# argsim/argsim

Measured on AMD Instinct MI355X. Metric: sentences/sec per ELBO step, higher is better.
Workload: dtype f32; 1 GPU; BASELINE configs[1]: 1xMI355X fp32, latent_dim 128, vocab 8k, seq_len 64, batch 256 per GPU; FULL synthetic Zipf batches, dim_emb 512, 3 layers, step 20000; global_batch=256, seq_len=64, parallelism=dp1, gru=persistent

## Files before the change

### argsim_amd/csrc/ctx.h

```cpp
#pragma once
#include "../../include/argsim_vae.h"
#include "kernels.h"

#include <fcntl.h>
#include <sys/file.h>
#include <unistd.h>

#include <algorithm>
#include <cmath>
#include <cstdio>
#include <cstring>
#include <string>
#include <vector>

#pragma GCC visibility push(hidden)
namespace avae { namespace host {

struct ParamEntry {
    std::string name;
    int64_t offset;
    int ndim;
    int64_t shape[4];
    int g16;
    int bucket;
// ... 7 lines not shown
struct avae_ctx {
    avae_config cfg{};
    int device = 0;
    hipStream_t stream = nullptr;
    std::string err;
    std::vector<avae::host::ParamEntry> params;
    int64_t numel = 0;
    std::vector<std::pair<int64_t, int64_t>> buckets;
    float *P = nullptr, *G = nullptr, *M = nullptr, *Vv = nullptr;
    int64_t step = 0;
    avae_grad_hook hook = nullptr; void* hook_user = nullptr;
    std::vector<int> hook_pending;
    int persistent = 1;
    bool first_step_checked = false;
    int gru_ablate = 0, gru_force_slow = 0, gru_stagger = 0, gru_item = 2;
    int skinny = 1;
    int score_plan[4] = {0, 0, 0, 0};
    const int* expect_ptr[3] = {nullptr, nullptr, nullptr}; int expect_val[3] = {0, 0, 0};
    int compact = 2;
    int skip_pad = 1;
    int shared_device = 0; int lock_fd = -1;
    int dyn_split = 1;
    int dyn_thin = 1;
    int enc_top1 = 1;
    int table_l1 = 1;
    int bf16_act = 1;
    int bf16_sv = 1;
    int bf16_tn = 1;
    int logits16 = 1;
    int bf16_nt8 = 1;
    int bf16_direct = 0;
    int gru_spec = 2;
    int gru_ring = 1;
    int bwd_rs = 2;
    int knn_chunk = 0;
    int agg_chunk = 0;
    int ward_form = 0;
    int probe_chunk = 0;
    int gru_bf16 = 1;
    int64_t oE = 0, oKout = 0, oBout = 0, oWmu = 0, oBmu = 0, oWlv = 0, oBlv = 0, oWex = 0, oBex = 0;
    std::vector<avae::host::GruP> enc;
    std::vector<avae::host::GruP> dec;
    float* losses = nullptr;
    float* acc = nullptr;
    int* errw = nullptr;
    unsigned* counters = nullptr;
    float* scratch = nullptr;
    int64_t scratch_n = 0;
    char* ws = nullptr; size_t ws_cap = 0;
    int B = 0, Ss = 0, St = 0;
    int timing = 0, timing_on = 0;
    unsigned short *bfA = nullptr, *bfB = nullptr; size_t bfA_cap = 0, bfB_cap = 0;
    float* slab = nullptr; size_t slab_floats = 0;
    unsigned short* bfP = nullptr; size_t bfP_cap = 0;
    struct Stamp { hipEvent_t a, b; int cls; double flops; const int* dyn; int dyn_max; };
    std::vector<Stamp> stamps; size_t stamps_used = 0;
    int32_t* hint_dev = nullptr; volatile int32_t* hint_host = nullptr;
    const int32_t *cnt_src = nullptr, *cnt_tgt = nullptr;
};

#pragma GCC visibility push(hidden)
namespace avae { namespace host {

#define AV_CHECK(expr)                                                                              \
    do { hipError_t e_ = (expr); if (e_ != hipSuccess) {                                            \
        char b_[512]; snprintf(b_, sizeof b_, "%s:%d: %s -> %s", __FILE__, __LINE__, #expr, hipGetErrorString(e_)); \
        h->err = b_; return 1; } } while (0)
#define AV_TRY(expr) do { int r_ = (expr); if (r_) return r_; } while (0)

inline int fail(avae_ctx* h, const std::string& m) { h->err = m; return 1; }

#define AV_GRU(expr)                                                                                                \
    do { hipError_t e_ = (expr);                                                                                    \
         if (e_ == hipErrorCooperativeLaunchTooLarge)                                                               \
             return fail(h, "persistent GRU kernel: its workgroups cannot all be resident on this device at once (occupancy query x CU count < grid); " \
                            "run with avae_set_option(\"persistent\", 0)");                                         \
         if (e_ != hipSuccess) { char b_[512]; snprintf(b_, sizeof b_, "%s:%d: %s -> %s", __FILE__, __LINE__, #expr, hipGetErrorString(e_)); \
             h->err = b_; return 1; } } while (0)

struct DeviceTurn {
    avae_ctx* h; bool held = false;
    explicit DeviceTurn(avae_ctx* h_) : h(h_) {
        if (!h->shared_device || !h->persistent) return;
        if (h->lock_fd < 0) {
            char path[64]; snprintf(path, sizeof path, "/tmp/argsim_vae_dev%d.lock", h->device);
            h->lock_fd = open(path, O_CREAT | O_RDWR, 0666);
        }
        if (h->lock_fd >= 0 && flock(h->lock_fd, LOCK_EX) == 0) held = true;
    }
    ~DeviceTurn() { if (held) { (void)hipStreamSynchronize(h->stream); (void)flock(h->lock_fd, LOCK_UN); } }
};
// ... 10 lines not shown
        s = &h->stamps[h->stamps_used++];
        s->cls = cls; s->flops = flops; s->dyn = dyn; s->dyn_max = dyn_max;
        (void)hipEventRecord(s->a, h->stream);
    }
    ~Timed() { if (s) (void)hipEventRecord(s->b, h->stream); }
};

struct Ws {
    int32_t *src_tm, *lens_src, *lens_tgt, *lead, *gold, *rank, *cidx, *ntok, *pred;
    float *emb_src, *emb_tgt, *ew, *dew;
    std::vector<float*> e_gi, e_hs, e_sv[2], e_hp[2];
    std::vector<float*> d_gi, d_hd, d_sv, d_hp;
    float *hpick, *mu, *lv, *z, *eps, *kld, *h0;
    float *xlast, *gib, *svb, *dgib, *dghb, *dxl;
    float *hc, *ho, *logits;
    float *loss_samp, *errt_samp;
    float *dho, *dhc, *dhd[2], *dgi_d, *dgh_d, *dh0, *carry, *dh0sum, *dz, *dmu, *dlv, *dhpick;
    float *dhs[2], *dgi_e, *dgh_e, *demb_src, *demb_tgt;
    std::vector<unsigned short*> e_hs16, d_hd16, e_hp16[2], d_hp16;
    std::vector<char> act_e, act_d, acth_e, acth_d;
    std::vector<unsigned short*> x16_e, x16_d;
    const unsigned short* x16_kept_e(int i) const { return x16_valid ? x16_e[i] : nullptr; }
    const unsigned short* x16_kept_d(int i) const { return x16_valid ? x16_d[i] : nullptr; }
    bool x16_valid = false;
    unsigned short *dgi16_d, *dgh16_d, *dgi16_e, *dgh16_e;
    int32_t* scat;
    int32_t *grp_src, *grp_tgt;
    int32_t *tokrow_src, *tokrow_tgt;
    float* xbuf; size_t xbuf_floats;
    int32_t *ord_perm[3], *ord_slens[3]; int ord_T[3], ord_cpj[3]; bool ord_ok[3];
    int32_t *map_src, *nact_src, *nsrc; bool compact;
    int32_t *map_tgt, *nact_tgt, *ntgt; bool compact_d;
    int Bx;
    int bx_enc() const { return compact ? Bx : 0; }
    int bx_dec() const { return compact_d ? Bx : 0; }
};

struct Bump {
    char* base; size_t off = 0;
    template <class T> T* take(size_t n) {
        off = (off + 255) & ~(size_t)255;
        T* p = base ? reinterpret_cast<T*>(base + off) : nullptr;
        off += n * sizeof(T);
        return p;
    }
    template <class T> T* opt(bool on, size_t n) { return on ? take<T>(n) : nullptr; }
};

struct Pair { const float* A; const float* B; float* C; const float* bias; };

struct GemmCall {
    const float* A; int lda; bool a_mc;
    const float* B; int ldb; bool b_nc;
    float* C; int ldc;
    int M, N, K;
    float alpha = 1.f; const float* bias = nullptr; int accumulate = 0;
    const int* dyn = nullptr; int dyn_kind = 0;
    const Pair* pair = nullptr;
    bool wgrad = false;
    bool allow_atomic = false;
    bool rows_are_batch = false;
    int thin = -1, split_k = 0;
    const unsigned short* A16 = nullptr; const unsigned short* B16 = nullptr;
    unsigned short* keep_a16 = nullptr;
    unsigned short* c16 = nullptr;

// ... 78 lines not shown
```

### argsim_amd/csrc/handle.cpp

```cpp
#include "ctx.h"

using namespace avae;
using namespace avae::host;

static std::string g_create_err;

namespace avae { namespace host {

int grow_scratch(avae_ctx* h, size_t need, const char* what)
{
    if (h->scratch_n >= (int64_t)need) return 0;
    AV_CHECK(hipStreamSynchronize(h->stream));
    if (h->scratch) AV_CHECK(hipFree(h->scratch));
    h->scratch = nullptr; h->scratch_n = 0;
    if (hipMalloc(reinterpret_cast<void**>(&h->scratch), need) != hipSuccess) {
        (void)hipGetLastError();
        h->scratch = nullptr;
        char b_[256]; snprintf(b_, sizeof b_, "%s: %.0f MB of scratch could not be allocated on the device", what, (double)need / 1048576.0);
        return fail(h, b_);
    }
    h->scratch_n = (int64_t)need;
    return 0;
}

// ... 189 lines not shown
    if (!base) return fail(h, "bad tensor kind");
    float* flat = base + e->offset;
    int64_t n = e->shape[0] * e->shape[1] * e->shape[2] * e->shape[3];
    if (!e->g16) {
        AV_CHECK(hipMemcpyAsync(get ? buf : flat, get ? flat : buf, n * sizeof(float), hipMemcpyDeviceToDevice, h->stream));
    } else {
        int D = h->cfg.dim_emb, cols = (int)(e->ndim == 2 ? e->shape[1] : 1);
        if (get) AV_CHECK(g16_permute(h->stream, buf, flat, D, cols, false));
        else     AV_CHECK(g16_permute(h->stream, flat, buf, D, cols, true));
    }
    return 0;
}
int avae_get_tensor(avae_handle h, const char* name, int kind, float* buf) { return xfer_tensor(h, name, kind, buf, true); }
int avae_set_tensor(avae_handle h, const char* name, int kind, const float* buf) { return xfer_tensor(h, name, kind, const_cast<float*>(buf), false); }

int avae_get_step(avae_handle h, int64_t* s) { if (!h || !s) return 1; *s = h->step; return 0; }
int avae_set_step(avae_handle h, int64_t s) { if (!h) return 1; h->step = s; return 0; }

int avae_set_grad_hook(avae_handle h, avae_grad_hook hook, void* user) { if (!h) return 1; h->hook = hook; h->hook_user = user; return 0; }

int avae_set_option(avae_handle h, const char* key, int value)
{
    if (!h || !key) return 1;
    if (!strcmp(key, "persistent")) { h->persistent = value; return 0; }
    if (!strcmp(key, "gru_item")) { h->gru_item = value; return 0; }
    if (!strcmp(key, "gru_stagger")) { h->gru_stagger = value; return 0; }
    if (!strcmp(key, "gru_force_slow")) { h->gru_force_slow = value; return 0; }
    if (!strcmp(key, "gru_bf16")) { h->gru_bf16 = value != 0; return 0; }
    if (!strcmp(key, "bwd_rs")) { h->bwd_rs = value; return 0; }
    if (!strcmp(key, "dyn_split")) { h->dyn_split = value != 0; return 0; }
    if (!strcmp(key, "shared_device")) { h->shared_device = value != 0; return 0; }
    if (!strcmp(key, "gru_spec")) { h->gru_spec = value; return 0; }
    if (!strcmp(key, "gru_ring")) { h->gru_ring = value != 0; return 0; }
    if (!strcmp(key, "bf16_nt8")) { h->bf16_nt8 = value != 0; return 0; }
    if (!strcmp(key, "logits16")) { h->logits16 = value != 0; return 0; }
    if (!strcmp(key, "bf16_direct")) { h->bf16_direct = value != 0; return 0; }
    if (!strcmp(key, "bf16_tn")) { h->bf16_tn = value != 0; return 0; }
    if (!strcmp(key, "bf16_sv")) { h->bf16_sv = value != 0; return 0; }
    if (!strcmp(key, "bf16_act")) { h->bf16_act = value != 0; return 0; }
    if (!strcmp(key, "table_l1")) { h->table_l1 = value != 0; return 0; }
    if (!strcmp(key, "enc_top1")) { h->enc_top1 = value != 0; return 0; }
    if (!strcmp(key, "dyn_thin")) { h->dyn_thin = value != 0; return 0; }
    if (!strcmp(key, "skip_pad")) { h->skip_pad = value != 0; return 0; }
    if (!strcmp(key, "compact")) { h->compact = value; return 0; }
    if (!strcmp(key, "skinny")) { h->skinny = value; return 0; }
    if (!strcmp(key, "knn_chunk")) { if (value < 0) return fail(h, "knn_chunk must be >= 0"); h->knn_chunk = value; return 0; }
    if (!strcmp(key, "agg_chunk")) { if (value < 0) return fail(h, "agg_chunk must be >= 0"); h->agg_chunk = value; return 0; }
    if (!strcmp(key, "ward_form")) { if (value < 0 || value > 2) return fail(h, "ward_form must be 0 (planner), 1 (one-workgroup) or 2 (launch-per-merge)"); h->ward_form = value; return 0; }
    if (!strcmp(key, "probe_chunk")) { if (value < 0) return fail(h, "probe_chunk must be >= 0"); h->probe_chunk = value; return 0; }
    if (!strcmp(key, "gru_ablate")) {
        if (value && !gru_diag_build()) return fail(h, "gru_ablate needs the diagnostic build of libargsim_vae.so (make -C argsim_amd/csrc DIAG=1)");
        h->gru_ablate = value; return 0;
    }
    if (!strcmp(key, "timing")) { h->timing = value; h->timing_on = value; h->stamps_used = 0; return 0; }
    if (!strcmp(key, "timing_pause")) { h->timing = value ? 0 : h->timing_on; return 0; }
    return fail(h, "unknown option");
}
int avae_timing_collect(avae_handle h, double* out)
{
    if (!h || !out) return 1;
    AV_CHECK(hipStreamSynchronize(h->stream));
    for (int i = 0; i < 9; ++i) out[i] = 0.0;
    std::vector<std::pair<const int*, int>> seen;
    for (size_t i = 0; i < h->stamps_used; ++i) {
        float ms = 0.f;
        AV_CHECK(hipEventElapsedTime(&ms, h->stamps[i].a, h->stamps[i].b));
// ... 17 lines not shown
```

### argsim_amd/csrc/hooks.cpp

```cpp
#include "ctx.h"

using namespace avae;
using namespace avae::host;

extern "C" {

int avae_debug_team_batch(int32_t B) { return B > 0 ? gru_team_batch(B) : 0; }
int avae_debug_gemm_plan(const int32_t* in, int32_t n, int32_t* out)
{
    if (!in || !out || n < 0) return 1;
    for (int r = 0; r < n; ++r, in += 19, out += 15) {
        const GemmShape s{in[0] != 0, in[1] != 0, in[2], in[3], in[4], in[5], in[6], in[7], in[8], in[9], in[10], in[11] != 0, in[12] != 0,
                          in[13] != 0, in[14] != 0, in[15], in[16] != 0, in[17] != 0, in[18] != 0};
        const GemmPlan p = gemm_plan(s);
        out[0] = p.n;
        for (int i = 0; i < 2; ++i) {
            const GemmLaunch l = i < p.n ? p.launch[i] : GemmLaunch{0, 0, 0, 0, 0, 0, 0};
            const int32_t f[7] = {l.row0, l.rows, l.thin, l.split_k, l.accumulate, l.zero, l.dyn};
            std::copy(f, f + 7, out + 1 + 7 * i);
        }
    }
    return 0;
}
int avae_debug_gemm_call(avae_handle h, int a_mc, int b_nc, const float* A, const float* Bm, float* Cm, const float* bias, int M, int N, int K,
// ... 41 lines not shown
                     pair ? other : nullptr, pair ? other : nullptr, nullptr, nullptr};
    const GemmF32Form f = gemm_f32_form(a_mc != 0, b_nc != 0, g);
    const int32_t v[8] = {f.tile, f.fast, f.db, f.persist, (int32_t)f.gx, (int32_t)f.gy, (int32_t)f.gz, f.err != hipSuccess};
    std::copy(v, v + 8, out);
    return 0;
}
int avae_debug_score_plan(avae_handle h, int32_t out[4])
{
    if (!h || !out) return 1;
    for (int i = 0; i < 4; ++i) out[i] = h->score_plan[i];
    return 0;
}
int avae_debug_present_ids(avae_handle h, int32_t out[2])
{
    if (!h || !out) return 1;
    AV_CHECK(hipStreamSynchronize(h->stream));
    out[0] = out[1] = -1;
    if (h->cnt_src) AV_CHECK(hipMemcpy(&out[0], h->cnt_src, sizeof(int), hipMemcpyDeviceToHost));
    if (h->cnt_tgt) AV_CHECK(hipMemcpy(&out[1], h->cnt_tgt, sizeof(int), hipMemcpyDeviceToHost));
    return 0;
}
int avae_debug_train_ce(avae_handle h, float* out, int32_t max_n, int32_t* n_out)
{
    if (!h || !out || !n_out) return 1;
    if (h->B < 1) return fail(h, "avae_debug_train_ce: no training forward has run on this handle");
    Ws w;
    AV_TRY(get_ws(h, w, h->B, h->Ss, h->St, true));
    int n = 0;
    AV_CHECK(hipMemcpyAsync(&n, w.ntok, sizeof(int), hipMemcpyDeviceToHost, h->stream));
    AV_CHECK(hipStreamSynchronize(h->stream));
    n = std::min(n, (int)max_n);
    AV_CHECK(hipMemcpyAsync(out, w.loss_samp, (size_t)n * sizeof(float), hipMemcpyDeviceToDevice, h->stream));
    *n_out = n;
    return 0;
}
int avae_debug_timing(avae_handle h, double* out, int max_n, int* n)
{
    if (!h || !out || !n) return 1;
    AV_CHECK(hipStreamSynchronize(h->stream));
    *n = (int)std::min<size_t>(h->stamps_used, (size_t)max_n);
    std::vector<std::pair<const int*, int>> seen;
    for (int i = 0; i < *n; ++i) {
        float ms = 0.f;
        AV_CHECK(hipEventElapsedTime(&ms, h->stamps[i].a, h->stamps[i].b));
        double f = 1.0;
        AV_TRY(dyn_fraction(h, h->stamps[i], seen, &f));
        const double fl = h->stamps[i].flops * f;
        out[3 * i] = h->stamps[i].cls; out[3 * i + 1] = ms; out[3 * i + 2] = fl;
    }
    return 0;
}
int avae_debug_stamps(avae_handle h, unsigned long long* out)
{
    if (!h || !out) return 1;
    AV_CHECK(hipStreamSynchronize(h->stream));
    AV_CHECK(hipMemcpy(out, h->errw + 16, 32 * sizeof(unsigned long long), hipMemcpyDeviceToHost));
    AV_CHECK(hipMemset(h->errw + 16, 0, 32 * sizeof(unsigned long long)));
    return 0;
}
int avae_debug_gemm(avae_handle h, int a_mc, int b_nc, const float* A, const float* Bm, float* Cm, const float* bias,
                    int M, int N, int K, int lda, int ldb, int ldc, float alpha, int accumulate, int split_k)
{
    if (!h) return 1;
    GemmCall c{A, lda, a_mc != 0, Bm, ldb, b_nc != 0, Cm, ldc, M, N, K};
    c.alpha = alpha; c.bias = bias; c.accumulate = accumulate;
    return gemm(h, c.form(split_k == -3 ? 3 : (split_k < 0 ? 1 : (split_k >= 1000 ? 2 : 0)), split_k < 0 ? 1 : (split_k >= 1000 ? split_k - 1000 : split_k)));
// ... 203 lines not shown
```

### argsim_amd/csrc/kernels.h

```cpp
#pragma once
#include <hip/hip_runtime.h>
#include <stdint.h>

#include "gemm_plan.h"

namespace avae {

struct GemmArgs {
    const float* A; const float* B; float* C; const float* bias;
    int M, N, K, lda, ldb, ldc;
    float alpha;
    int accumulate;
    int split_k;
    const int* dyn; int dyn_kind;
    int dyn_expect;
    int thin;
    const float* A2; const float* B2; float* C2; const float* bias2;
    float* slab = nullptr; size_t slab_floats = 0;
    unsigned short* c16 = nullptr;
    int nt8 = 1;
};
hipError_t gemm_f32(hipStream_t st, bool a_mc, bool b_nc, const GemmArgs& g);
struct GemmF32Form { int tile; bool fast, db, persist; unsigned gx, gy, gz; hipError_t err; };
GemmF32Form gemm_f32_form(bool a_mc, bool b_nc, const GemmArgs& g);
// ... 81 lines not shown
hipError_t gru_bwd_rs_launch(hipStream_t st, const GruArgs& a, const GruPlan& p);
hipError_t gru_fwd_team_launch(hipStream_t st, const GruArgs& a, const GruPlan& p);
hipError_t gru_bwd_team_launch(hipStream_t st, const GruArgs& a, const GruPlan& p);
hipError_t gru_reg_launch(hipStream_t st, const GruArgs& a, bool fwd, int grid, bool need_resident);
hipError_t gru_fwd_item_launch(hipStream_t st, const GruArgs& a, int grid);
hipError_t gru_first_step_fwd(hipStream_t st, const float* gi, const float* bR, float* h_out, int ldo, float* sv, int B, int D, const int32_t* lens = nullptr);
hipError_t gru_first_step_bwd(hipStream_t st, const float* dh, int ldd, const float* sv, float* dgi, float* dgh, int B, int D, const int32_t* lens = nullptr);
bool gru_diag_build();

struct PrepArgs {
    const int32_t* src; const int32_t* tgt;
    int B, Ss, St, eos, bos;
    int train; float keepwd; uint64_t seed; const uint8_t* keep_mask;
    int32_t* src_tm;
    int32_t* lens_src;
    int32_t* lens_tgt;
    int32_t* lead;
    int32_t* gold;
    int32_t* rank;
    int32_t* cidx;
    int32_t* ntok;
    float* zero2;
    int32_t* chunk_counts;
};
constexpr int kPrepChunks = 1024;
hipError_t prep_ids(hipStream_t st, const PrepArgs& p);

hipError_t embed_gather(hipStream_t st, const float* E, const int32_t* ids, float* out, int n, int D, int V);
hipError_t embed_scatter_add2(hipStream_t st, float* dE, const int32_t* ids0, const float* dout0, int n0, const int32_t* ids1,
                              const float* dout1, int n1, int D, int V, int32_t* scratch);
bool id_groups_supported(int V);
inline size_t id_groups_ints(size_t n, size_t V) { return 4 * V + 2 + n + (n / 32 + V + 1) + 2 * V + 4; }
hipError_t id_groups_build(hipStream_t st, const int32_t* ids, int n, int V, int32_t* scratch, bool lists);
const int32_t* id_groups_rank(int32_t* scratch, int n, int V);
const int32_t* id_groups_uid(int32_t* scratch, int n, int V);
const int32_t* id_groups_count(int32_t* scratch, int n, int V);
hipError_t rank_rows(hipStream_t st, int32_t* out, const int32_t* ids, const int32_t* rank, int n, int V);
hipError_t rows_gather_ranked(hipStream_t st, float* dst, const float* src, const int32_t* ids, const int32_t* rank, int n, int W, int V);
hipError_t rows_group_sum(hipStream_t st, float* dst, const int32_t* ids, const float* src, int n, int W, int V, int32_t* scratch);
hipError_t rows_add_indexed(hipStream_t st, float* dst, const float* src, const int32_t* uid, const int32_t* nuniq, int n_max, int D);
inline size_t embed_scatter_scratch_ints(size_t n, size_t V) { return 4 * V + 2 + n + (n / 32 + V + 1); }
struct RowOrder { const int32_t* lens; int add, T, cpj; int32_t* perm; int32_t* slens; };
hipError_t row_order(hipStream_t st, const RowOrder* orders, int n, int Breal, int B, int S, int32_t* steps_sum = nullptr, int sum_rows = 0);
hipError_t rows_gather(hipStream_t st, float* dst, const float* src, const int32_t* idx, const int32_t* n_dev, int n_max, int D, const int32_t* map = nullptr);
hipError_t rows_expand(hipStream_t st, float* dst, const float* src, const int32_t* rank, int rows, int D, const int32_t* map = nullptr);
hipError_t pick_last(hipStream_t st, float* h, const float* hs, const int32_t* lens, int B, int W, const int32_t* map = nullptr);
hipError_t pick_last16(hipStream_t st, float* h, const unsigned short* hs16, const int32_t* lens, int B, int W, const int32_t* map = nullptr);
hipError_t pick_last_add(hipStream_t st, float* dhs, const float* d, const int32_t* lens, int B, int W, const int32_t* map = nullptr);
hipError_t row_map(hipStream_t st, const int32_t* lens, int add, int S, int B, int32_t* map, int32_t* nact, int32_t* count);
hipError_t zero_rows_dyn(hipStream_t st, float* X, const int32_t* count, int rows_max, int W);
hipError_t pick_last_bwd(hipStream_t st, float* dhs, const float* dh, const int32_t* lens, int S, int B, int W);

hipError_t latent_fwd(hipStream_t st, const float* mu, const float* lv, const float* eps_in, float* eps_out, float* z,
                      float* kld, int n, int train, uint64_t seed, float free_bits, float* acc);
hipError_t latent_bwd(hipStream_t st, const float* dz, const float* mu, const float* lv, const float* eps_used,
                      float* dmu, float* dlv, int B, int R, float coef, float free_bits);

struct CeArgs {
    float* logits;
    const int32_t* gold;
    const int32_t* cidx;
    const int32_t* n_dev;
    int n_max, V;
    int write_grad; float inv_n;
    float* loss_samp; float* errt_samp; int32_t* pred;
    float* loss_acc;
// ... 163 lines not shown
```

### argsim_amd/csrc/model.cpp

```cpp
#include "ctx.h"

using namespace avae;

namespace avae { namespace host {

static bool phantom_batch(const avae_ctx* h, int B)
{
    return h->compact && h->skip_pad && h->persistent && h->cfg.dim_emb == 512 && gru_team_batch(B) > B;
}
bool use_table(const avae_ctx* h, int rows, int B)
{
    if (!h->table_l1 || !id_groups_supported(h->cfg.dim_tgt)) return false;
    return rows >= h->cfg.dim_tgt || (rows >= 1024 && phantom_batch(h, B));
}

void layout(avae_ctx* h, Bump& b, Ws& w, int B, int Ss, int St, bool train)
{
    const int D = h->cfg.dim_emb, V = h->cfg.dim_tgt, R = h->cfg.dim_rep, L = h->cfg.rnn_layers;
    const size_t T = St + 1, rs = (size_t)Ss * B, rt = T * B;
    w.src_tm = b.take<int32_t>(rs); w.lens_src = b.take<int32_t>(B); w.lens_tgt = b.take<int32_t>(B);
    w.lead = b.take<int32_t>(rt); w.gold = b.take<int32_t>(rt); w.rank = b.take<int32_t>(rt);
    w.cidx = b.take<int32_t>(rt); w.ntok = b.take<int32_t>(4 + kPrepChunks); w.pred = b.take<int32_t>(rt);
    w.emb_src = b.take<float>(rs * D); w.emb_tgt = b.take<float>(rt * D);
    const bool tab_s = use_table(h, (int)rs, B), tab_t = use_table(h, (int)rt, B);
// ... 363 lines not shown
    AV_CHECK(row_map(h->stream, w.lens_tgt, 1, T, B, w.map_tgt, w.nact_tgt, w.ntgt));
    w.compact_d = true;
    return 0;
}
int build_compact_dec(avae_ctx* h, Ws& w, int B, int T)
{
    w.compact = false; w.compact_d = false;
    h->expect_ptr[0] = h->expect_ptr[1] = h->expect_ptr[2] = nullptr;
    if (!h->compact || h->compact == 3 || !h->persistent || T < 2 || !use_table(h, T * B, B)) return 0;
    if (w.Bx == B || !w.ord_ok[2]) return 0;
    GruArgs q{};
    gru_common(h, w, q, 1, T, B, 3 * h->cfg.dim_emb, h->cfg.dim_emb, nullptr, w.Bx);
    if (!gru_plan(q, true, true).full()) return 0;
    AV_CHECK(row_map(h->stream, w.lens_tgt, 1, T, B, w.map_tgt, w.nact_tgt, w.ntgt));
    w.compact_d = true;
    return 0;
}

static int run_encoder(avae_ctx* h, Ws& w, int B, int Ss, bool save)
{
    const int D = h->cfg.dim_emb, V = h->cfg.dim_tgt, L = h->cfg.rnn_layers;
    const int rs = Ss * B;
    const bool table = use_table(h, rs, B);
    h->cnt_src = table ? id_groups_count(w.grp_src, rs, V) : nullptr;
    const int32_t* const cdyn = w.compact ? w.nsrc : nullptr;
    const int32_t* const cmap = w.compact ? w.map_src : nullptr;
    if (!table) AV_CHECK(embed_gather(h->stream, h->P + h->oE, w.src_tm, w.emb_src, rs, D, V));
    const float* x = w.emb_src; int In = D;
    for (int i = 0; i < L; ++i) {
        const GruP& p = h->enc[i];
        const bool top1 = i == L - 1 && top_one_step(h);
        if (i == 0 && table) {
            const int32_t* cnt = id_groups_count(w.grp_src, rs, V);
            AV_CHECK(id_groups_build(h->stream, w.src_tm, rs, V, w.grp_src, save));
            AV_CHECK(rows_gather(h->stream, w.emb_src, h->P + h->oE, id_groups_uid(w.grp_src, rs, V), cnt, std::min(V, rs), D));
            AV_TRY(gemm(h, nt(w.emb_src, D, h->P + p.W, D, w.ew, 6 * D, std::min(V, rs), 6 * D, D).biased(h->P + p.bW).rows(cnt)));
        } else if (i > 0 && w.act_e[i - 1]) {
            AV_TRY(gemm_bf16_pre(h, nt(nullptr, In, h->P + p.W, In, w.e_gi[i], 6 * D, rs, top1 ? 3 * D : 6 * D, In).a16(w.e_hs16[i - 1]).biased(h->P + p.bW).rows(cdyn)));
        } else {
        AV_TRY(gemm(h, nt(x, In, h->P + p.W, In, w.e_gi[i], 6 * D, rs, top1 ? 3 * D : 6 * D, In).biased(h->P + p.bW).rows(cdyn).keep(save ? w.x16_e[i] : nullptr)));
        }
        GruArgs a{};
        gru_common(h, w, a, top1 ? 1 : 2, Ss, B, 6 * D, 2 * D, w.lens_src, w.bx_enc());
        const bool table0 = i == 0 && table, indirect = table0 && gru_plan(a, true, h->persistent != 0).form == GruForm::team;
        if (indirect) AV_CHECK(rank_rows(h->stream, w.tokrow_src, w.src_tm, id_groups_rank(w.grp_src, rs, V), rs, V));
        else if (table0) AV_CHECK(rows_gather_ranked(h->stream, w.e_gi[0], w.ew, w.src_tm, id_groups_rank(w.grp_src, rs, V), rs, 6 * D, V));
        for (int d = 0; d < a.njobs; ++d) {
            GruJob& j = a.job[d];
            j.gi = (indirect ? w.ew : w.e_gi[i]) + d * 3 * D;
            j.gi_rows = indirect ? w.tokrow_src : nullptr;
            j.R = h->P + p.R + (int64_t)d * 3 * D * D;
            j.bR = h->P + p.bR + d * 3 * D;
            j.h0 = nullptr;
            j.hs = w.e_hs[i] + d * D;
            j.sv = save ? w.e_sv[d][i] : nullptr;
            j.hp = save ? w.e_hp[d][i] : nullptr;
            j.reverse = d;
        }
        attach_sv16(h, a, save);
        if (w.e_hs16[i] && tn16_ok(h, 3 * D, D) && both_team_bf16(h, a, save)) {
            w.act_e[i] = 1; w.acth_e[i] = 1;
            for (int d = 0; d < a.njobs; ++d) { a.job[d].hs16 = w.e_hs16[i] + d * D; a.job[d].hp16 = w.e_hp16[d][i]; }
        }
        attach_order(h, w, a, true, top1 ? 1 : 0);
        a.rowmap = cmap;
        a.spec = spec_pick(h);
        { Timed t(h, 1, 2.0 * a.njobs * Ss * (double)B * D * 3 * D);
// ... 10 lines not shown
    }
    if (w.act_e[L - 1]) AV_CHECK(pick_last16(h->stream, w.hpick, w.e_hs16[L - 1], w.lens_src, B, 2 * D, cmap));
    else
    AV_CHECK(pick_last(h->stream, w.hpick, w.e_hs[L - 1], w.lens_src, B, 2 * D, cmap));
    if (top_one_step(h))
        AV_CHECK(gru_first_step_fwd(h->stream, w.gib, h->P + h->enc[L - 1].bR + 3 * D, w.hpick + D, 2 * D, save ? w.svb : nullptr, B, D, w.lens_src));
    return 0;
}

static int run_latent(avae_ctx* h, Ws& w, int B, bool train, uint64_t seed, const float* eps)
{
    const int D = h->cfg.dim_emb, R = h->cfg.dim_rep;
    {
        const Pair lv{w.hpick, h->P + h->oWlv, w.lv, h->P + h->oBlv};
        AV_TRY(gemm(h, nn(w.hpick, 2 * D, h->P + h->oWmu, R, w.mu, R, B, R, 2 * D).biased(h->P + h->oBmu).with(&lv)));
    }
    AV_CHECK(latent_fwd(h->stream, w.mu, w.lv, eps, w.eps, w.z, w.kld, B * R, train ? 1 : 0, seed, h->cfg.free_bits, nullptr));
    return 0;
}

int run_decoder_rnn(avae_ctx* h, Ws& w, int B, int T, const float* state_in, int64_t state_stride, bool save, const int32_t* ids0, bool compact, const int32_t* share_rows, int share_n)
{
    const int32_t* const cdyn = compact ? w.ntgt : nullptr;
    const int32_t* const cmap = compact ? w.map_tgt : nullptr;
    const int D = h->cfg.dim_emb, L = h->cfg.rnn_layers;
    const int rt = T * B;
    const float* x = w.emb_tgt;
    h->cnt_tgt = ids0 ? id_groups_count(w.grp_tgt, rt, h->cfg.dim_tgt) : nullptr;
    for (int i = 0; i < L; ++i) {
        const GruP& p = h->dec[i];
        if (i == 0 && ids0) {
            const int V = h->cfg.dim_tgt;
            const int32_t* cnt = id_groups_count(w.grp_tgt, rt, V);
            AV_CHECK(id_groups_build(h->stream, ids0, rt, V, w.grp_tgt, save));
            AV_CHECK(rows_gather(h->stream, w.emb_tgt, h->P + h->oE, id_groups_uid(w.grp_tgt, rt, V), cnt, std::min(V, rt), D));
            AV_TRY(gemm(h, nt(w.emb_tgt, D, h->P + p.W, D, w.ew, 3 * D, std::min(V, rt), 3 * D, D).biased(h->P + p.bW).rows(cnt)));
        } else if (i == 0 && share_rows) {
            AV_TRY(gemm(h, nt(x, D, h->P + p.W, D, w.d_gi[0], 3 * D, share_n, 3 * D, D).biased(h->P + p.bW)));
        } else if (i > 0 && w.act_d[i - 1]) {
            AV_TRY(gemm_bf16_pre(h, nt(nullptr, D, h->P + p.W, D, w.d_gi[i], 3 * D, rt, 3 * D, D).a16(w.d_hd16[i - 1]).biased(h->P + p.bW).rows(cdyn)));
        } else {
        AV_TRY(gemm(h, nt(x, D, h->P + p.W, D, w.d_gi[i], 3 * D, rt, 3 * D, D).biased(h->P + p.bW).rows(cdyn).keep(save ? w.x16_d[i] : nullptr)));
        }
        GruArgs a{};
        gru_common(h, w, a, 1, T, B, 3 * D, D, nullptr, compact ? w.Bx : 0);
        GruJob& j = a.job[0];
        const bool table0 = i == 0 && ids0, indirect = table0 && gru_plan(a, true, h->persistent != 0).form == GruForm::team;
        if (indirect) AV_CHECK(rank_rows(h->stream, w.tokrow_tgt, ids0, id_groups_rank(w.grp_tgt, rt, h->cfg.dim_tgt), rt, h->cfg.dim_tgt));
        else if (table0) AV_CHECK(rows_gather_ranked(h->stream, w.d_gi[0], w.ew, ids0, id_groups_rank(w.grp_tgt, rt, h->cfg.dim_tgt), rt, 3 * D, h->cfg.dim_tgt));
        j.gi = indirect ? w.ew : w.d_gi[i]; j.gi_rows = indirect ? w.tokrow_tgt : nullptr;
        if (i == 0 && share_rows) j.gi_rows = share_rows;
        j.R = h->P + p.R; j.bR = h->P + p.bR;
        j.h0 = state_in + state_stride * i;
        j.hs = w.d_hd[i];
        j.sv = save ? w.d_sv[i] : nullptr;
        j.hp = save ? w.d_hp[i] : nullptr;
        j.reverse = 0;
        attach_sv16(h, a, save);
        if (w.d_hp16[i] && tn16_ok(h, 3 * D, D) && both_team_bf16(h, a, save)) {
            if (i < L - 1) { w.act_d[i] = 1; j.hs16 = w.d_hd16[i]; }
            w.acth_d[i] = 1; j.hp16 = w.d_hp16[i];
        }
        if (T > 1) attach_order(h, w, a, true, 2);
        a.rowmap = cmap;
        a.spec = spec_pick(h);
        { Timed t(h, 1, 2.0 * T * (double)B * D * 3 * D);
          DeviceTurn turn(h);
          AV_GRU(gru_forward(h->stream, a, h->persistent != 0)); }
        x = w.d_hd[i];
    }
    return 0;
}

static int forward(avae_ctx* h, Ws& w, const int32_t* src, const int32_t* tgt, int B, int Ss, int St, bool train,
            uint64_t seed, const uint8_t* keep_mask, const float* eps, float inv_n)
{
    const int D = h->cfg.dim_emb, V = h->cfg.dim_tgt, R = h->cfg.dim_rep;
    const int T = St + 1, rt = T * B;
    Sched sc = schedule(h);
    PrepArgs p = prep_from_ws(w);
    p.src = src; p.tgt = tgt; p.B = B; p.Ss = Ss; p.St = St; p.eos = h->cfg.eos; p.bos = h->cfg.bos;
    p.train = train ? 1 : 0; p.keepwd = sc.keepwd; p.seed = seed; p.keep_mask = keep_mask;
    AV_CHECK(prep_ids(h->stream, p));
    AV_TRY(build_row_orders(h, w, B, Ss, T, true));
    AV_TRY(build_compact(h, w, B, Ss, T, train));
    AV_TRY(run_encoder(h, w, B, Ss, train));
    AV_TRY(run_latent(h, w, B, train, seed, eps));
    AV_TRY(gemm(h, nn(w.z, R, h->P + h->oWex, D, w.h0, D, B, D, R).biased(h->P + h->oBex).batch_rows()));
    if (use_table(h, rt, B)) AV_TRY(run_decoder_rnn(h, w, B, T, w.h0, 0, train, w.lead, w.compact_d));
    else {
        AV_CHECK(embed_gather(h->stream, h->P + h->oE, w.lead, w.emb_tgt, rt, D, V));
        AV_TRY(run_decoder_rnn(h, w, B, T, w.h0, 0, train));
    }
    AV_TRY(run_logits_ce(h, w, rt, train, inv_n));
    float beta = h->cfg.kl_beta;
    AV_CHECK(finalize_losses(h->stream, h->losses, w.loss_samp, w.ntok, rt, w.kld, B * R, h->cfg.free_bits, 1.f / ((float)B * R), sc.anneal * beta));
    return 0;
}

int run_logits_ce(avae_ctx* h, Ws& w, int rt, bool train, float inv_n)
{
    const int D = h->cfg.dim_emb, V = h->cfg.dim_tgt, L = h->cfg.rnn_layers;
    AV_CHECK(rows_gather(h->stream, w.hc, w.d_hd[L - 1], w.cidx, w.ntok, rt, D, w.compact_d ? w.map_tgt : nullptr));
    AV_TRY(gemm(h, nn(w.hc, D, h->P + h->oKout, D, w.ho, D, rt, D, D).biased(h->P + h->oBout).rows(w.ntok)));
    CeArgs c{};
    c.logits = w.logits; c.gold = w.gold; c.cidx = w.cidx; c.n_dev = w.ntok; c.n_max = rt; c.V = V;
    c.write_grad = train ? 1 : 0; c.inv_n = inv_n;
    if (train && h->cfg.compute_dtype == 1 && (V & 7) == 0) {
        AV_TRY(grow_bf16(h, &h->bfP, &h->bfP_cap, (size_t)rt * V));
        c.grad16 = h->bfP;
        if (h->logits16 && !h->bf16_direct && gemm_bf16_c16_takes(rt, V, D, w.ntok, h->bf16_nt8)) c.logits16 = 1;
    }
    GemmCall lg = nt(w.ho, D, h->P + h->oE, D, w.logits, V, rt, V, D).scaled(1.f / sqrtf((float)D)).rows(w.ntok);
    if (c.logits16) lg.form(0).c16 = h->bfP;
    AV_TRY(gemm(h, lg));
    c.loss_samp = w.loss_samp; c.errt_samp = w.errt_samp; c.pred = w.pred; c.loss_acc = nullptr;
    AV_CHECK(softmax_ce(h->stream, c));
    return 0;
// ... 335 lines not shown
```

### argsim_amd/csrc/ops.hip

```cpp
#include <algorithm>
#include "kernels.h"
#include "mfma_tile.h"
#include "reduce_dev.h"
#include "sample_dev.h"

namespace avae {


__device__ __forceinline__ bool prep_kept(const PrepArgs& p, int i)
{
    const int t = i / p.B, b = i - t * p.B;
    return t == 0 || p.tgt[(size_t)b * p.St + t - 1] != p.eos;
}
__device__ __forceinline__ int block_sum256(int v, int* red)
{
    v = wave_sum(v);
    if ((threadIdx.x & 63) == 0) red[threadIdx.x >> 6] = v;
    __syncthreads();
    const int s = red[0] + red[1] + red[2] + red[3];
    __syncthreads();
    return s;
}
__global__ __launch_bounds__(256) void prep_ids_kernel(PrepArgs p, int per, int nchunks)
{
// ... 262 lines not shown
        return hipGetLastError();
    }
    Scatter2 a{dE, ids0, dout0, n0, ids1, dout1, n1, D, V, scratch, scratch + V, scratch + 2 * V, scratch + 3 * V + 1, scratch + 4 * V + 2, scratch + 4 * V + 2 + n, nullptr, nullptr, nullptr};
    hipError_t e = zero_fill(st, scratch, sizeof(int32_t) * 2 * (size_t)V);
    if (e != hipSuccess) return e;
    const int blocks = (n + kScatterTok - 1) / kScatterTok;
    hipLaunchKernelGGL(scatter_hist_kernel, dim3(blocks), dim3(256), 0, st, a);
    hipLaunchKernelGGL(scatter_scan_kernel, dim3(1), dim3(1024), 0, st, a);
    hipLaunchKernelGGL(scatter_fill_kernel, dim3(blocks), dim3(256), 0, st, a);
    hipLaunchKernelGGL(scatter_reduce_kernel, dim3(std::min((n / 4 + V + 3) / 4, 4096)), dim3(256), 0, st, a);
    return hipGetLastError();
}

static Scatter2 id_groups_view(const int32_t* ids, int n, int V, int32_t* scratch)
{
    int32_t* rank = scratch + 4 * (size_t)V + 2 + n + ((size_t)n / kScatterSeg + V + 1);
    return Scatter2{nullptr, ids, nullptr, n, nullptr, nullptr, 0, 0, V, scratch, scratch + V, scratch + 2 * V, scratch + 3 * V + 1,
                    scratch + 4 * V + 2, scratch + 4 * (size_t)V + 2 + n, rank, rank + V, rank + 2 * (size_t)V};
}
const int32_t* id_groups_rank(int32_t* scratch, int n, int V) { return id_groups_view(nullptr, n, V, scratch).rank; }
const int32_t* id_groups_uid(int32_t* scratch, int n, int V) { return id_groups_view(nullptr, n, V, scratch).uid; }
const int32_t* id_groups_count(int32_t* scratch, int n, int V) { return id_groups_view(nullptr, n, V, scratch).nuniq; }
bool id_groups_supported(int V) { return V <= kScatterLdsV; }
hipError_t id_groups_build(hipStream_t st, const int32_t* ids, int n, int V, int32_t* scratch, bool lists)
{
    if (n <= 0 || V > kScatterLdsV) return hipErrorInvalidValue;
    Scatter2 a = id_groups_view(ids, n, V, scratch);
    hipError_t e = zero_fill(st, scratch, sizeof(int32_t) * 2 * (size_t)V);
    if (e != hipSuccess) return e;
    const int blocks = (n + kScatterTok - 1) / kScatterTok;
    hipLaunchKernelGGL(scatter_hist_kernel, dim3(blocks), dim3(256), 0, st, a);
    hipLaunchKernelGGL(scatter_scan_kernel, dim3(1), dim3(1024), 0, st, a);
    if (lists) hipLaunchKernelGGL(scatter_fill_kernel, dim3(blocks), dim3(256), 0, st, a);
    return hipGetLastError();
}
__global__ __launch_bounds__(256) void rows_gather_ranked_kernel(float* __restrict__ dst, const float* __restrict__ src,
                                                                 const int32_t* __restrict__ ids, const int32_t* __restrict__ rank, int n, int W, int V)
{
    const int lane = threadIdx.x & 63, wpb = blockDim.x >> 6;
    for (int row = blockIdx.x * wpb + (threadIdx.x >> 6); row < n; row += gridDim.x * wpb) {
        int id = ids[row];
        id = id < 0 ? 0 : (id >= V ? V - 1 : id);
        const float4* s = reinterpret_cast<const float4*>(src + (size_t)rank[id] * W);
        float4* d = reinterpret_cast<float4*>(dst + (size_t)row * W);
        for (int c = lane; c < W / 4; c += 64) d[c] = s[c];
    }
}
__global__ __launch_bounds__(256) void rank_rows_kernel(int32_t* __restrict__ out, const int32_t* __restrict__ ids, const int32_t* __restrict__ rank, int n, int V)
{
    for (int t = blockIdx.x * 256 + threadIdx.x; t < n; t += gridDim.x * 256) {
        int id = ids[t];
        id = id < 0 ? 0 : (id >= V ? V - 1 : id);
        out[t] = rank[id];
    }
}
hipError_t rank_rows(hipStream_t st, int32_t* out, const int32_t* ids, const int32_t* rank, int n, int V)
{
    if (n <= 0) return hipSuccess;
    hipLaunchKernelGGL(rank_rows_kernel, dim3(std::min((n + 255) / 256, 2048)), dim3(256), 0, st, out, ids, rank, n, V);
    return hipGetLastError();
}
hipError_t rows_gather_ranked(hipStream_t st, float* dst, const float* src, const int32_t* ids, const int32_t* rank, int n, int W, int V)
{
    if (n <= 0) return hipSuccess;
    if (W & 3) return hipErrorInvalidValue;
    hipLaunchKernelGGL(rows_gather_ranked_kernel, dim3(std::min((n + 3) / 4, 8192)), dim3(256), 0, st, dst, src, ids, rank, n, W, V);
// ... 827 lines not shown
```

### argsim_amd/lib.py

```python
import ctypes as C
import os
import subprocess

_HERE = os.path.dirname(os.path.abspath(__file__))
LIB_PATH = os.path.join(_HERE, 'libargsim_vae.so')
CSRC = os.path.join(_HERE, 'csrc')


def source_digest():
    import glob
    import hashlib
    h = hashlib.sha1()
    files = sorted(glob.glob(os.path.join(CSRC, '*.hip')) + glob.glob(os.path.join(CSRC, '*.cpp')) + glob.glob(os.path.join(CSRC, '*.h')))
    files.append(os.path.join(os.path.dirname(_HERE), 'include', 'argsim_vae.h'))
    for f in files:
        h.update(os.path.basename(f).encode())
        with open(f, 'rb') as fh:
            h.update(fh.read())
    return h.hexdigest()[:16]


class AvaeConfig(C.Structure):
    _fields_ = [('dim_tgt', C.c_int32), ('dim_emb', C.c_int32), ('dim_rep', C.c_int32), ('rnn_layers', C.c_int32),
                ('accelerate', C.c_float), ('learn_rate', C.c_float), ('bos', C.c_int32), ('eos', C.c_int32),
# ... 65 lines not shown
    'avae_eval': (C.c_int, [_P, _P, _P, C.c_int32, C.c_int32, C.c_int32, _P, _P, _P, C.POINTER(C.c_int32)]),
    'avae_encode': (C.c_int, [_P, _P, C.c_int32, C.c_int32, _P, _P]),
    'avae_decode_init': (C.c_int, [_P, _P, C.c_int32, _P]),
    'avae_decode_step': (C.c_int, [_P, _P, _P, C.c_int32, _P, _P]),
    'avae_decode_greedy': (C.c_int, [_P, _P, C.c_int32, C.c_int32, _P, C.POINTER(C.c_int32)]),
    'avae_decode_sample': (C.c_int, [_P, _P, C.c_int32, C.c_int32, C.POINTER(AvaeSampleConfig), _P, _P, C.POINTER(C.c_int32)]),
    'avae_decode_sample_p': (C.c_int, [_P, _P, C.c_int32, C.c_int32, C.POINTER(AvaeSamplePConfig), _P, _P, _P, C.POINTER(C.c_int32)]),
    'avae_decode_beam': (C.c_int, [_P, _P, C.c_int32, C.c_int32, C.POINTER(AvaeBeamConfig), _P, _P, _P, _P, _P, _P, _P, C.POINTER(C.c_int32)]),
    'avae_score': (C.c_int, [_P, _P, _P, C.c_int32, C.c_int32, C.c_int32, C.POINTER(AvaeScoreConfig), _P, _P, _P, _P, _P, _P]),
    'avae_score_z': (C.c_int, [_P, _P, _P, C.c_int32, C.c_int32, _P, _P]),
    'avae_knn': (C.c_int, [_P, _P, C.c_int32, _P, C.c_int32, C.c_int32, C.POINTER(AvaeKnnConfig), _P, _P]),
    'avae_agg_logq': (C.c_int, [_P, _P, C.c_int32, _P, _P, C.c_int32, C.c_int32, C.POINTER(AvaeAggConfig), _P, _P]),
    'avae_latent_moments': (C.c_int, [_P, _P, _P, C.c_int32, C.c_int32, _P]),
    'avae_probe_fit': (C.c_int, [_P, _P, C.c_int32, C.c_int32, _P, C.c_int32, C.POINTER(AvaeProbeConfig), _P, _P]),
    'avae_probe_decision': (C.c_int, [_P, _P, C.c_int32, C.c_int32, _P, C.c_int32, _P]),
    'avae_probe_fit_l1': (C.c_int, [_P, _P, C.c_int32, C.c_int32, _P, C.c_int32, C.POINTER(AvaeProbeL1Config), _P, _P]),
    'avae_ward': (C.c_int, [_P, _P, C.c_int32, C.POINTER(C.c_int32), C.c_int32, C.POINTER(AvaeWardConfig), _P, _P, _P]),
    'avae_ward_cut': (C.c_int, [_P, _P, C.POINTER(C.c_int32), C.c_int32, C.POINTER(C.c_int32), _P]),
    'avae_set_option': (C.c_int, [_P, C.c_char_p, C.c_int]),
    'avae_debug_gemm': (C.c_int, [_P, C.c_int, C.c_int, _P, _P, _P, _P] + [C.c_int] * 6 + [C.c_float, C.c_int, C.c_int]),
    'avae_debug_gemm_dyn': (C.c_int, [_P, _P, _P, _P, C.c_int, C.c_int, C.c_int, _P]),
    'avae_debug_gemm_c16': (C.c_int, [_P, _P, _P, _P, C.c_int, C.c_int, C.c_int, C.c_float, _P]),
    'avae_debug_gemm_tn16': (C.c_int, [_P, _P, _P, _P] + [C.c_int] * 6 + [C.c_float]),
    'avae_debug_softmax_ce': (C.c_int, [_P, _P, _P, C.c_int, _P, _P, _P, C.c_int, C.c_int, C.c_int, C.c_float, _P, _P, _P, C.POINTER(C.c_int)]),
    'avae_debug_argmax_rows': (C.c_int, [_P, _P, _P, C.c_int, C.c_int]),
    'avae_debug_op': (C.c_int, [_P, C.c_char_p, C.POINTER(_P), C.POINTER(C.c_int64), C.POINTER(C.c_float)]),
    'avae_debug_op_layout': (C.c_int, [C.c_int64, C.c_int64, C.POINTER(C.c_int64)]),
    'avae_debug_sample_rows': (C.c_int, [_P, _P, C.c_int, C.c_int, C.c_int, C.POINTER(AvaeSampleConfig), _P, _P]),
    'avae_debug_sample_rows_p': (C.c_int, [_P, _P, C.c_int, C.c_int, C.c_int, C.POINTER(AvaeSamplePConfig), _P, _P, _P, _P]),
    'avae_debug_beam_select': (C.c_int, [_P, _P, C.c_int, C.c_int, C.c_int, _P, _P, _P, _P, _P, _P]),
    'avae_timing_collect': (C.c_int, [_P, C.POINTER(C.c_double)]),
    'avae_debug_timing': (C.c_int, [_P, C.POINTER(C.c_double), C.c_int, C.POINTER(C.c_int)]),
    'avae_debug_train_ce': (C.c_int, [_P, _P, C.c_int32, C.POINTER(C.c_int32)]),
    'avae_debug_stamps': (C.c_int, [_P, C.POINTER(C.c_uint64)]),
    'avae_debug_present_ids': (C.c_int, [_P, C.POINTER(C.c_int32)]),
    'avae_debug_score_plan': (C.c_int, [_P, C.POINTER(C.c_int32)]),
    'avae_debug_team_batch': (C.c_int, [C.c_int32]),
    'avae_debug_gemm_plan': (C.c_int, [_P, C.c_int32, _P]),
    'avae_debug_gemm_call': (C.c_int, [_P, C.c_int, C.c_int, _P, _P, _P, _P] + [C.c_int] * 6 + [C.c_float, C.c_int, C.c_int, _P, C.c_int, _P, _P, _P, _P]),
    'avae_debug_gemm_forced': (C.c_int, [_P, C.c_int, C.c_int, _P, _P, _P, _P] + [C.c_int] * 6 + [C.c_float, C.c_int, C.c_int, C.c_int, _P, C.c_int, C.c_int,
                                         _P, _P, _P, _P]),
    'avae_debug_gemm_f32_form': (C.c_int, [C.c_int] * 14 + [C.POINTER(C.c_int32)]),
    'avae_debug_gru_plan': (C.c_int, [C.POINTER(C.c_int64), C.c_int, C.c_int, C.POINTER(C.c_int64)]),
    'avae_debug_gru': (C.c_int, [_P, C.c_int, C.c_int, C.POINTER(C.c_int64), C.POINTER(_P), C.POINTER(_P), C.POINTER(C.c_int64)]),
    'avae_bucket_count': (C.c_int, [_P]),
    'avae_bucket_info': (C.c_int, [_P, C.c_int, C.POINTER(C.c_int64), C.POINTER(C.c_int64)]),
}

_lib = None


def build(force=False, jobs=4):
    if force:
        subprocess.run(['make', '-C', CSRC, 'clean'], check=True, stdout=subprocess.DEVNULL)
    subprocess.run(['make', '-C', CSRC, '-j%d' % jobs], check=True, stdout=subprocess.DEVNULL)
    return LIB_PATH


def load():
    global _lib
    if _lib is not None:
        return _lib
    if not os.path.exists(LIB_PATH):
        raise RuntimeError("libargsim_vae.so is not built: run `python -c 'import __graft_entry__ as g; g.build()'` "
                           "(there is no CPU fallback for the HIP path)")
    lib = C.CDLL(LIB_PATH)
# ... 7 lines not shown
```

Before: 15900 sentences/sec.

## Fuse id-group histogram, scan and list build into one LDS kernel for both sources

Replaces the three-kernel id grouping (global histogram, single-block scan, scatter fill) with one 1024-thread kernel. It keeps the histogram in shared memory and builds the per-id token lists with an in-LDS radix sort. When both the source and target embedding tables are used, the target grouping is built in the same launch as a second block, which removes several small launches and global atomics per step. The cost is a single workgroup per source doing serial scan work, with a large LDS footprint that is capped by a fits check.

```diff
diff --git a/argsim_amd/csrc/ctx.h b/argsim_amd/csrc/ctx.h
--- a/argsim_amd/csrc/ctx.h
+++ b/argsim_amd/csrc/ctx.h
@@ -63,6 +63,7 @@
     int bf16_direct = 0;
     int gru_spec = 2;
     int gru_ring = 1;
+    int id_groups_fused = 1;
     int bwd_rs = 2;
     int knn_chunk = 0;
     int agg_chunk = 0;
@@ -88,6 +89,7 @@
     std::vector<Stamp> stamps; size_t stamps_used = 0;
     int32_t* hint_dev = nullptr; volatile int32_t* hint_host = nullptr;
     const int32_t *cnt_src = nullptr, *cnt_tgt = nullptr;
+    int last_groups_fused = 0;
 };
 
 #pragma GCC visibility push(hidden)
@@ -164,6 +166,7 @@
     int32_t *map_src, *nact_src, *nsrc; bool compact;
     int32_t *map_tgt, *nact_tgt, *ntgt; bool compact_d;
     int Bx;
+    int pair_rt = -1; bool groups_built = false;
     int bx_enc() const { return compact ? Bx : 0; }
     int bx_dec() const { return compact_d ? Bx : 0; }
 };
diff --git a/argsim_amd/csrc/handle.cpp b/argsim_amd/csrc/handle.cpp
--- a/argsim_amd/csrc/handle.cpp
+++ b/argsim_amd/csrc/handle.cpp
@@ -245,6 +245,7 @@
     if (!strcmp(key, "shared_device")) { h->shared_device = value != 0; return 0; }
     if (!strcmp(key, "gru_spec")) { h->gru_spec = value; return 0; }
     if (!strcmp(key, "gru_ring")) { h->gru_ring = value != 0; return 0; }
+    if (!strcmp(key, "id_groups_fused")) { h->id_groups_fused = value != 0; return 0; }
     if (!strcmp(key, "bf16_nt8")) { h->bf16_nt8 = value != 0; return 0; }
     if (!strcmp(key, "logits16")) { h->logits16 = value != 0; return 0; }
     if (!strcmp(key, "bf16_direct")) { h->bf16_direct = value != 0; return 0; }
diff --git a/argsim_amd/csrc/hooks.cpp b/argsim_amd/csrc/hooks.cpp
--- a/argsim_amd/csrc/hooks.cpp
+++ b/argsim_amd/csrc/hooks.cpp
@@ -97,6 +97,20 @@
     n = std::min(n, (int)max_n);
     AV_CHECK(hipMemcpyAsync(out, w.loss_samp, (size_t)n * sizeof(float), hipMemcpyDeviceToDevice, h->stream));
     *n_out = n;
+    return 0;
+}
+int avae_debug_id_groups(avae_handle h, const int32_t* ids0, const int32_t* ids1, int n0, int n1, int V, int32_t* scratch0, int32_t* scratch1, int32_t* form_out)
+{
+    if (!h || !form_out) return 1;
+    if (!ids0) { *form_out = h->last_groups_fused; return 0; }
+    if (!scratch0 || (ids1 && !scratch1)) return fail(h, "avae_debug_id_groups: a scratch per source");
+    const bool fused = h->id_groups_fused && id_groups_fused_fits(n0, V) && (!ids1 || id_groups_fused_fits(n1, V));
+    *form_out = fused ? (ids1 ? 2 : 1) : 0;
+    if (fused) AV_CHECK(id_groups_build_fused(h->stream, ids0, n0, scratch0, ids1, n1, scratch1, V, true));
+    else {
+        AV_CHECK(id_groups_build(h->stream, ids0, n0, V, scratch0, true));
+        if (ids1) AV_CHECK(id_groups_build(h->stream, ids1, n1, V, scratch1, true));
+    }
     return 0;
 }
 int avae_debug_timing(avae_handle h, double* out, int max_n, int* n)
diff --git a/argsim_amd/csrc/kernels.h b/argsim_amd/csrc/kernels.h
--- a/argsim_amd/csrc/kernels.h
+++ b/argsim_amd/csrc/kernels.h
@@ -137,6 +137,8 @@
 bool id_groups_supported(int V);
 inline size_t id_groups_ints(size_t n, size_t V) { return 4 * V + 2 + n + (n / 32 + V + 1) + 2 * V + 4; }
 hipError_t id_groups_build(hipStream_t st, const int32_t* ids, int n, int V, int32_t* scratch, bool lists);
+bool id_groups_fused_fits(int n, int V);
+hipError_t id_groups_build_fused(hipStream_t st, const int32_t* ids0, int n0, int32_t* scratch0, const int32_t* ids1, int n1, int32_t* scratch1, int V, bool lists);
 const int32_t* id_groups_rank(int32_t* scratch, int n, int V);
 const int32_t* id_groups_uid(int32_t* scratch, int n, int V);
 const int32_t* id_groups_count(int32_t* scratch, int n, int V);
diff --git a/argsim_amd/csrc/model.cpp b/argsim_amd/csrc/model.cpp
--- a/argsim_amd/csrc/model.cpp
+++ b/argsim_amd/csrc/model.cpp
@@ -419,7 +419,17 @@
         const bool top1 = i == L - 1 && top_one_step(h);
         if (i == 0 && table) {
             const int32_t* cnt = id_groups_count(w.grp_src, rs, V);
-            AV_CHECK(id_groups_build(h->stream, w.src_tm, rs, V, w.grp_src, save));
+            w.groups_built = false;
+            if (w.pair_rt > 0) {
+                AV_CHECK(id_groups_build_fused(h->stream, w.src_tm, rs, w.grp_src, w.lead, w.pair_rt, w.grp_tgt, V, save));
+                w.groups_built = true; h->last_groups_fused = 2;
+            } else if (w.pair_rt < 0 && h->id_groups_fused && id_groups_fused_fits(rs, V)) {
+                AV_CHECK(id_groups_build_fused(h->stream, w.src_tm, rs, w.grp_src, nullptr, 0, nullptr, V, save));
+                h->last_groups_fused = 1;
+            } else {
+                AV_CHECK(id_groups_build(h->stream, w.src_tm, rs, V, w.grp_src, save));
+                h->last_groups_fused = 0;
+            }
             AV_CHECK(rows_gather(h->stream, w.emb_src, h->P + h->oE, id_groups_uid(w.grp_src, rs, V), cnt, std::min(V, rs), D));
             AV_TRY(gemm(h, nt(w.emb_src, D, h->P + p.W, D, w.ew, 6 * D, std::min(V, rs), 6 * D, D).biased(h->P + p.bW).rows(cnt)));
         } else if (i > 0 && w.act_e[i - 1]) {
@@ -496,7 +506,14 @@
         if (i == 0 && ids0) {
             const int V = h->cfg.dim_tgt;
             const int32_t* cnt = id_groups_count(w.grp_tgt, rt, V);
-            AV_CHECK(id_groups_build(h->stream, ids0, rt, V, w.grp_tgt, save));
+            if (w.groups_built) {}
+            else if (w.pair_rt < 0 && h->id_groups_fused && id_groups_fused_fits(rt, V)) {
+                AV_CHECK(id_groups_build_fused(h->stream, ids0, rt, w.grp_tgt, nullptr, 0, nullptr, V, save));
+                h->last_groups_fused = 1;
+            } else {
+                AV_CHECK(id_groups_build(h->stream, ids0, rt, V, w.grp_tgt, save));
+                h->last_groups_fused = 0;
+            }
             AV_CHECK(rows_gather(h->stream, w.emb_tgt, h->P + h->oE, id_groups_uid(w.grp_tgt, rt, V), cnt, std::min(V, rt), D));
             AV_TRY(gemm(h, nt(w.emb_tgt, D, h->P + p.W, D, w.ew, 3 * D, std::min(V, rt), 3 * D, D).biased(h->P + p.bW).rows(cnt)));
         } else if (i == 0 && share_rows) {
@@ -548,6 +565,7 @@
     AV_CHECK(prep_ids(h->stream, p));
     AV_TRY(build_row_orders(h, w, B, Ss, T, true));
     AV_TRY(build_compact(h, w, B, Ss, T, train));
+    w.pair_rt = h->id_groups_fused && use_table(h, Ss * B, B) && use_table(h, rt, B) && id_groups_fused_fits(Ss * B, V) && id_groups_fused_fits(rt, V) ? rt : 0;
     AV_TRY(run_encoder(h, w, B, Ss, train));
     AV_TRY(run_latent(h, w, B, train, seed, eps));
     AV_TRY(gemm(h, nn(w.z, R, h->P + h->oWex, D, w.h0, D, B, D, R).biased(h->P + h->oBex).batch_rows()));
diff --git a/argsim_amd/csrc/ops.hip b/argsim_amd/csrc/ops.hip
--- a/argsim_amd/csrc/ops.hip
+++ b/argsim_amd/csrc/ops.hip
@@ -318,6 +318,119 @@
     hipLaunchKernelGGL(scatter_hist_kernel, dim3(blocks), dim3(256), 0, st, a);
     hipLaunchKernelGGL(scatter_scan_kernel, dim3(1), dim3(1024), 0, st, a);
     if (lists) hipLaunchKernelGGL(scatter_fill_kernel, dim3(blocks), dim3(256), 0, st, a);
+    return hipGetLastError();
+}
+constexpr int kGroupsIpt = 20;
+constexpr size_t kGroupsLdsLimit = 160 * 1024;
+static size_t id_groups_bins_bytes(int V) { return std::max<size_t>(4 * (size_t)V, 16 * 1024 * sizeof(unsigned short)); }
+static size_t id_groups_lds_bytes(int n, int V) { return id_groups_bins_bytes(V) + 64 + 3 * sizeof(unsigned short) * (((size_t)n + 7) & ~(size_t)7); }
+bool id_groups_fused_fits(int n, int V)
+{
+    return n >= 1 && V >= 1 && V <= kScatterLdsV && n <= kGroupsIpt * 1024 && id_groups_lds_bytes(n, V) <= kGroupsLdsLimit;
+}
+struct IdGroups2 { Scatter2 s[2]; int lists; };
+__global__ __launch_bounds__(1024) void id_groups_lds_kernel(IdGroups2 g)
+{
+    extern __shared__ __attribute__((aligned(16))) unsigned char gl[];
+    const Scatter2& a = g.s[blockIdx.x];
+    const int n = a.n0, V = a.V, tid = threadIdx.x;
+    const size_t binb = max((size_t)4 * V, (size_t)(16 * 1024 * sizeof(unsigned short))), np = ((size_t)n + 7) & ~(size_t)7;
+    int* const bins = reinterpret_cast<int*>(gl);
+    unsigned short* const cnt16 = reinterpret_cast<unsigned short*>(gl);
+    int* const wsum = reinterpret_cast<int*>(gl + binb);
+    unsigned short* const ids16 = reinterpret_cast<unsigned short*>(gl + binb + 64);
+    unsigned short* const tokA = ids16 + np;
+    unsigned short* const tokB = tokA + np;
+    for (int i = tid; i < V; i += 1024) bins[i] = 0;
+    __syncthreads();
+    for (int t = tid; t < n; t += 1024) { const int id = scatter_id(a, t); ids16[t] = (unsigned short)id; atomicAdd(&bins[id], 1); }
+    __syncthreads();
+    for (int i = tid; i < V; i += 1024) { const int c = bins[i]; a.cnt[i] = c; a.cur[i] = g.lists ? c : 0; }
+    {
+        const int per = (V + 1023) / 1024, beg = min(V, tid * per), end = min(V, beg + per);
+        int tok = 0, seg = 0, uni = 0;
+        for (int i = beg; i < end; ++i) { const int c = bins[i]; tok += c; seg += (c + kScatterSeg - 1) / kScatterSeg; uni += c > 0; }
+        const int itok = block_scan1024(tok, wsum), iseg = block_scan1024(seg, wsum), iuni = block_scan1024(uni, wsum);
+        int rt = itok - tok, rs = iseg - seg, ru = iuni - uni;
+        for (int i = beg; i < end; ++i) {
+            const int c = bins[i];
+            a.off[i] = rt; a.segoff[i] = rs;
+            rt += c;
+            for (int k = (c + kScatterSeg - 1) / kScatterSeg; k > 0; --k) a.segid[rs++] = i;
+            if (a.rank) { a.rank[i] = c > 0 ? ru : -1; if (c > 0) a.uid[ru++] = i; }
+        }
+        if (tid == 1023) { a.off[V] = itok; a.segoff[V] = iseg; if (a.rank) a.nuniq[0] = iuni; }
+    }
+    if (!g.lists) return;
+    __syncthreads();
+    const int ipt = (n + 1023) / 1024, beg = tid * ipt;
+    int nbits = 0;
+    while (nbits < 31 && (1 << nbits) < V) ++nbits;
+    const unsigned short* src = nullptr;
+    unsigned short* dst = tokA;
+    for (int shift = 0; shift < nbits; shift += 4) {
+        int tok[kGroupsIpt], dr[kGroupsIpt];
+        unsigned c0 = 0u, c1 = 0u, c2 = 0u, c3 = 0u;
+#pragma unroll
+        for (int k = 0; k < kGroupsIpt; ++k) {
+            const int p = beg + k;
+            const bool live = k < ipt && p < n;
+            tok[k] = live ? (src ? (int)src[p] : p) : -1;
+        }
+#pragma unroll
+        for (int k = 0; k < kGroupsIpt; ++k) {
+            dr[k] = 0;
+            if (tok[k] < 0) continue;
+            const int d = ((int)ids16[tok[k]] >> shift) & 15, q = d >> 2, sh = 8 * (d & 3);
+            const unsigned one = 1u << sh, c = q == 0 ? c0 : (q == 1 ? c1 : (q == 2 ? c2 : c3));
+            dr[k] = d | ((int)((c >> sh) & 255u) << 4);
+            c0 += q == 0 ? one : 0u; c1 += q == 1 ? one : 0u; c2 += q == 2 ? one : 0u; c3 += q == 3 ? one : 0u;
+        }
+#pragma unroll
+        for (int d = 0; d < 16; ++d) cnt16[d * 1024 + tid] = (unsigned short)(((d < 4 ? c0 : (d < 8 ? c1 : (d < 12 ? c2 : c3))) >> (8 * (d & 3))) & 255u);
+        __syncthreads();
+        {
+            uint4* const my = reinterpret_cast<uint4*>(cnt16 + 16 * tid);
+            const uint4 lo = my[0], hi = my[1];
+            const unsigned w[8] = {lo.x, lo.y, lo.z, lo.w, hi.x, hi.y, hi.z, hi.w};
+            int s = 0;
+#pragma unroll
+            for (int q = 0; q < 8; ++q) s += (int)(w[q] & 0xffffu) + (int)(w[q] >> 16);
+            int run = block_scan1024(s, wsum) - s;
+            unsigned o[8];
+#pragma unroll
+            for (int q = 0; q < 8; ++q) {
+                const int a0 = run, a1 = run + (int)(w[q] & 0xffffu);
+                o[q] = (unsigned)a0 | ((unsigned)a1 << 16);
+                run = a1 + (int)(w[q] >> 16);
+            }
+            my[0] = make_uint4(o[0], o[1], o[2], o[3]); my[1] = make_uint4(o[4], o[5], o[6], o[7]);
+        }
+        __syncthreads();
+#pragma unroll
+        for (int k = 0; k < kGroupsIpt; ++k)
+            if (tok[k] >= 0) dst[(int)cnt16[(dr[k] & 15) * 1024 + tid] + (dr[k] >> 4)] = (unsigned short)tok[k];
+        __syncthreads();
+        src = dst; dst = dst == tokA ? tokB : tokA;
+    }
+    for (int t = tid; t < n; t += 1024) a.list[t] = src ? (int)src[t] : t;
+}
+hipError_t id_groups_build_fused(hipStream_t st, const int32_t* ids0, int n0, int32_t* scratch0, const int32_t* ids1, int n1, int32_t* scratch1, int V, bool lists)
+{
+    const bool two = ids1 != nullptr;
+    if (!id_groups_fused_fits(n0, V) || (two && !id_groups_fused_fits(n1, V))) return hipErrorInvalidValue;
+    static bool attr_done = false;
+    if (!attr_done) {
+        hipError_t e = hipFuncSetAttribute(reinterpret_cast<const void*>(id_groups_lds_kernel), hipFuncAttributeMaxDynamicSharedMemorySize, (int)kGroupsLdsLimit);
+        if (e != hipSuccess) return e;
+        attr_done = true;
+    }
+    IdGroups2 g{};
+    g.s[0] = id_groups_view(ids0, n0, V, scratch0);
+    g.s[1] = two ? id_groups_view(ids1, n1, V, scratch1) : g.s[0];
+    g.lists = lists ? 1 : 0;
+    const size_t lds = std::max(id_groups_lds_bytes(n0, V), two ? id_groups_lds_bytes(n1, V) : (size_t)0);
+    hipLaunchKernelGGL(id_groups_lds_kernel, dim3(two ? 2 : 1), dim3(1024), lds, st, g);
     return hipGetLastError();
 }
 __global__ __launch_bounds__(256) void rows_gather_ranked_kernel(float* __restrict__ dst, const float* __restrict__ src,
diff --git a/argsim_amd/lib.py b/argsim_amd/lib.py
--- a/argsim_amd/lib.py
+++ b/argsim_amd/lib.py
@@ -121,6 +121,7 @@
     'avae_timing_collect': (C.c_int, [_P, C.POINTER(C.c_double)]),
     'avae_debug_timing': (C.c_int, [_P, C.POINTER(C.c_double), C.c_int, C.POINTER(C.c_int)]),
     'avae_debug_train_ce': (C.c_int, [_P, _P, C.c_int32, C.POINTER(C.c_int32)]),
+    'avae_debug_id_groups': (C.c_int, [_P, _P, _P, C.c_int, C.c_int, C.c_int, _P, _P, C.POINTER(C.c_int32)]),
     'avae_debug_stamps': (C.c_int, [_P, C.POINTER(C.c_uint64)]),
     'avae_debug_present_ids': (C.c_int, [_P, C.POINTER(C.c_int32)]),
     'avae_debug_score_plan': (C.c_int, [_P, C.POINTER(C.c_int32)]),
```

Result: no change. 15910 sentences/sec, median of 3 (+0.1%).
